# SamSamhuns/face_detection_and_recognition

Measured on AMD Instinct MI355X. Metric: faces/sec end-to-end (detect->embed->cosine-filter), 576x1024 batch=256, higher is better.
Workload: dtype f32 (bf16x6 split GEMMs)

## Files before the change

face_detection_and_recognition_amd/csrc/capi.cpp:

```cpp
#include <stdarg.h>
#include <stdio.h>
#include <stdlib.h>
#include <string.h>

#include "common.h"

static thread_local char g_hip_err[256] = "";

void fp_set_hip_error(hipError_t e) {
  const char* s = hipGetErrorString(e);
  strncpy(g_hip_err, s ? s : "unknown", sizeof(g_hip_err) - 1);
  g_hip_err[sizeof(g_hip_err) - 1] = 0;
}

static fp_knobs read_knobs() {
  fp_knobs k;
  k.resize_per_pixel = getenv("FP_RESIZE_PER_PIXEL") != nullptr;
  return k;
}
static fp_knobs g_knobs = read_knobs();
const fp_knobs& fp_get_knobs() { return g_knobs; }

bool fp_dry_run(const fp_launch& L, const char* fmt, ...) {
  if (!L.dry) return false;
  if (L.name) {
    va_list ap;
    va_start(ap, fmt);
    vsnprintf(L.name, FP_KERNEL_NAME_MAX, fmt, ap);
    va_end(ap);
  }
  return true;
}

static int launch_op(const fp_op& op, const fp_launch& L) {
  switch (op.kind) {
    case FP_OP_CONV: return fp_launch_conv(op, L);
    case FP_OP_DWCONV: return fp_launch_dwconv(op, L);
    case FP_OP_MAXPOOL: return fp_launch_maxpool(op, L);
    case FP_OP_UPSAMPLE2X: return fp_launch_upsample2x(op, L);
    case FP_OP_COPY: return fp_launch_copy(op, L);
    case FP_OP_L2NORM: return fp_launch_l2norm(op, L);
    case FP_OP_BLAZEBLOCK: return fp_launch_blazeblock(op, L);
    case FP_OP_DWPW: return (op.flags & FP_OPF_SPLIT3) ? fp_launch_dwpwx6(op, L) : fp_launch_dwpw(op, L);
    case FP_OP_DWBLOCK: return (op.flags & FP_OPF_SPLIT3) ? fp_launch_dwblock_x6(op, L) : fp_launch_dwblock(op, L);
    case FP_OP_BLAZEPAIR: return op.stride == 2 ? fp_launch_blazepair_s2(op, L) : fp_launch_blazepair(op, L);
    case FP_OP_BLAZECHAIN: return fp_launch_blazechain(op, L);
    case FP_OP_SHUFDOWN: return fp_launch_shufdown(op, L);
    case FP_OP_SHUFUNIT: return fp_launch_shufunit(op, L);
    case FP_OP_YSTEM2: return fp_launch_ystem2(op, L);
    case FP_OP_YSTEM: return fp_launch_ystem(op, L);
    case FP_OP_YSTEM_U8: return fp_launch_ystem_u8(op, L);
    case FP_OP_STEM_U8: return fp_launch_stem_u8(op, L);
    case FP_OP_EMBED_HEAD: return fp_launch_embed_head(op, L);
    case FP_OP_POOL_LRN: return fp_launch_pool_lrn(op, L);
    case FP_OP_CLS_HEAD: return fp_launch_cls_head(op, L);
    default: return FP_ERR_UNSUPPORTED;
  }
}

static int dry_run(const fp_op& op, char* name) {
  const fp_launch L = {nullptr, nullptr, nullptr, 0, nullptr, true, name};
  return launch_op(op, L);
}

extern "C" {

int fp_abi_version(void) { return FP_ABI_VERSION; }

void fp_debug_reload_env(void) { g_knobs = read_knobs(); }

const char* fp_last_hip_error(void) { return g_hip_err; }

static unsigned fastdiv_host(unsigned n, fp_divisor d) { return (unsigned)(((unsigned long long)n * d.mul) >> 32) >> d.shift; }

int fp_selftest(void) {
  auto check = [&](unsigned d) -> bool {
    const fp_divisor dv = fp_make_divisor(d);
    const unsigned nmax = 0x7fffffffu, qmax = nmax / d;
    const unsigned qs[] = {0u, 1u, 2u, qmax / 3, qmax / 2, qmax - 1, qmax};
    for (unsigned q : qs) {
      const unsigned long long lo = (unsigned long long)q * d;
      const unsigned long long cand[] = {lo, lo + 1, lo + d - 1, lo + d / 2};
      for (unsigned long long n64 : cand) {
        if (n64 > nmax) continue;
        const unsigned n = (unsigned)n64;
        if (fastdiv_host(n, dv) != n / d) {
          snprintf(g_hip_err, sizeof(g_hip_err), "fp_fastdiv(%u, %u) = %u, expected %u", n, d, fastdiv_host(n, dv), n / d);
          return false;
        }
      }
    }
    if (fastdiv_host(nmax, dv) != nmax / d) {
      snprintf(g_hip_err, sizeof(g_hip_err), "fp_fastdiv(%u, %u) wrong at the top of the range", nmax, d);
      return false;
    }
    return true;
  };
  for (unsigned d = 2; d <= 4096; ++d)
    if (!check(d)) return FP_ERR_INVALID_ARG;
  const unsigned big[] = {4097u, 12321u, 16384u, 65535u, 65536u, 65537u, 1000003u, 16777216u, 123456789u, 1u << 30, (1u << 30) + 1u};
  for (unsigned d : big)
    if (!check(d)) return FP_ERR_INVALID_ARG;
  return FP_OK;
}

const char* fp_strerror(int status) {
  switch (status) {
    case FP_OK: return "ok";
    case FP_ERR_INVALID_ARG: return "invalid argument";
    case FP_ERR_BOUNDS: return "op touches memory outside the arena or weight blob";
    case FP_ERR_UNSUPPORTED: return "unsupported op or parameter combination";
    case FP_ERR_LAUNCH: return "HIP kernel launch failed";
    case FP_ERR_ALIGNMENT: return "channel count / stride / offset not a multiple of 4 floats";
    default: return "unknown status";
  }
}

static bool span_ok(int64_t off, int64_t extent, size_t limit) {
  return off >= 0 && extent >= 0 && (uint64_t)(off + extent) <= (uint64_t)limit;
}

static int validate_op(const fp_op& op, size_t weight_floats, size_t arena_floats) {
  if (op.N <= 0 || op.H <= 0 || op.W <= 0 || op.Cin <= 0) return FP_ERR_INVALID_ARG;
  const bool spatial = op.kind != FP_OP_L2NORM && op.kind != FP_OP_COPY;
  const int OH = spatial ? op.OH : op.H, OW = spatial ? op.OW : op.W;
  if (OH <= 0 || OW <= 0) return FP_ERR_INVALID_ARG;
  const bool ext_in = op.kind == FP_OP_YSTEM_U8 || op.kind == FP_OP_STEM_U8;
  const int Cout = (op.kind == FP_OP_CONV || op.kind == FP_OP_BLAZEBLOCK || op.kind == FP_OP_DWPW ||
                    op.kind == FP_OP_DWBLOCK || op.kind == FP_OP_BLAZEPAIR || op.kind == FP_OP_BLAZECHAIN || op.kind == FP_OP_YSTEM ||
                    op.kind == FP_OP_SHUFDOWN || op.kind == FP_OP_SHUFUNIT || op.kind == FP_OP_YSTEM2 || op.kind == FP_OP_EMBED_HEAD ||
                    op.kind == FP_OP_CLS_HEAD || ext_in) ? op.Cout : op.Cin;
  if (op.kind != FP_OP_DWBLOCK && op.kind != FP_OP_BLAZECHAIN && op.kind != FP_OP_SHUFDOWN && op.kind != FP_OP_SHUFUNIT &&
      op.kind != FP_OP_POOL_LRN && op.Cmid != 0)
    return FP_ERR_INVALID_ARG;
  if (op.kind == FP_OP_POOL_LRN && op.Cout != op.Cin) return FP_ERR_INVALID_ARG;
  if (op.row_lo != 0 || op.row_end != 0) {
    if (op.kind != FP_OP_BLAZEPAIR && op.kind != FP_OP_STEM_U8) return FP_ERR_UNSUPPORTED;
    if (op.row_lo < 0 || op.row_end <= op.row_lo || op.row_end > OH) return FP_ERR_INVALID_ARG;
  }
  if (Cout <= 0 || op.out_cmul < 1 || op.in_ld < op.Cin) return FP_ERR_INVALID_ARG;
  if (op.flags & ~(FP_OPF_IN_ROWPAD | FP_OPF_OUT_ROWPAD | FP_OPF_IN_C3 | FP_OPF_SPLIT3 | FP_OPF_IN_DW | FP_OPF_IN_UP2 | FP_OPF_OUT_DW |
                   FP_OPF_OUT_L2))
    return FP_ERR_INVALID_ARG;
  if ((op.flags & FP_OPF_OUT_L2) && op.kind != FP_OP_EMBED_HEAD) return FP_ERR_INVALID_ARG;
  if (op.flags & FP_OPF_OUT_DW) {
    if (op.kind != FP_OP_CONV) return FP_ERR_INVALID_ARG;
    if (!span_ok(op.slope_off, 13 * (int64_t)op.Cout, weight_floats)) return FP_ERR_BOUNDS;
    if (!span_ok(op.w_off, fp_stemdw_w_floats(op), weight_floats)) return FP_ERR_BOUNDS;
  }
  if (op.flags & FP_OPF_IN_UP2) {
    if (op.kind != FP_OP_CONV || !(op.flags & FP_OPF_SPLIT3)) return FP_ERR_INVALID_ARG;
    const int64_t up_ext = (int64_t)(op.N - 1) * op.res_ns + ((int64_t)op.res_H * op.res_W - 1) * op.res_ld + op.res_C;
    if (!span_ok(op.res_off, up_ext, arena_floats)) return FP_ERR_BOUNDS;
  }
  if ((op.flags & FP_OPF_IN_DW) && (op.kind != FP_OP_DWBLOCK || !(op.flags & FP_OPF_SPLIT3))) return FP_ERR_INVALID_ARG;
  if ((op.flags & FP_OPF_SPLIT3) && op.kind != FP_OP_DWBLOCK && op.kind != FP_OP_CONV && op.kind != FP_OP_DWPW && op.kind != FP_OP_BLAZECHAIN &&
      op.kind != FP_OP_SHUFDOWN && op.kind != FP_OP_SHUFUNIT && op.kind != FP_OP_YSTEM2 && op.kind != FP_OP_STEM_U8)
    return FP_ERR_INVALID_ARG;
  if ((op.flags & FP_OPF_IN_C3) && (op.Cin != 4 || (op.kind != FP_OP_CONV && op.kind != FP_OP_YSTEM)))
    return FP_ERR_INVALID_ARG;
  const bool in_rp = (op.flags & FP_OPF_IN_ROWPAD) != 0, out_rp = (op.flags & FP_OPF_OUT_ROWPAD) != 0;
  if (in_rp && op.kind != FP_OP_BLAZEBLOCK && op.kind != FP_OP_BLAZEPAIR) return FP_ERR_UNSUPPORTED;
  if (out_rp && !(op.kind == FP_OP_BLAZEBLOCK || op.kind == FP_OP_BLAZEPAIR || op.kind == FP_OP_STEM_U8 || op.kind == FP_OP_COPY ||
                  op.kind == FP_OP_CONV))
    return FP_ERR_UNSUPPORTED;
  if (out_rp && (op.out_cmul != 1 || op.out_ld != Cout)) return FP_ERR_UNSUPPORTED;
  if (op.kind == FP_OP_CONV || op.kind == FP_OP_DWCONV || op.kind == FP_OP_MAXPOOL || op.kind == FP_OP_BLAZEBLOCK ||
      op.kind == FP_OP_DWPW || op.kind == FP_OP_DWBLOCK || op.kind == FP_OP_BLAZEPAIR || op.kind == FP_OP_BLAZECHAIN ||
      op.kind == FP_OP_YSTEM || op.kind == FP_OP_SHUFDOWN || op.kind == FP_OP_SHUFUNIT || op.kind == FP_OP_YSTEM2 ||
      op.kind == FP_OP_POOL_LRN || ext_in) {
    if (op.KH <= 0 || op.KW <= 0 || op.stride <= 0 || op.pad_t < 0 || op.pad_l < 0) return FP_ERR_INVALID_ARG;
    if ((int64_t)(OH - 1) * op.stride - op.pad_t >= op.H || (int64_t)(OW - 1) * op.stride - op.pad_l >= op.W)
      return FP_ERR_INVALID_ARG;
  }
  if (op.kind == FP_OP_YSTEM2) {
    const int64_t res_ext = (int64_t)(op.N - 1) * op.res_ns + ((int64_t)op.OH * op.OW - 1) * op.res_ld + op.res_C;
    if (!span_ok(op.res_off, res_ext, arena_floats)) return FP_ERR_BOUNDS;
  }
  const int rc = dry_run(op, nullptr);
  if (rc != FP_OK) return rc;
  if (in_rp) {
    const int64_t lead = (int64_t)(op.W + 2) * op.in_ld;
    if (op.in_ns < ((int64_t)(op.H + 2) * (op.W + 1) + 1) * op.in_ld) return FP_ERR_INVALID_ARG;
    if (op.in_off < lead || !span_ok(op.in_off - lead, (int64_t)op.N * op.in_ns, arena_floats)) return FP_ERR_BOUNDS;
  } else {
    const int64_t in_ext = (int64_t)(op.N - 1) * op.in_ns + ((int64_t)op.H * op.W - 1) * op.in_ld + op.Cin;
    if (!ext_in && !span_ok(op.in_off, in_ext, arena_floats)) return FP_ERR_BOUNDS;
  }
  if (ext_in && op.in_off < 0) return FP_ERR_INVALID_ARG;
  const int64_t out_ch = ((op.kind == FP_OP_CONV || op.kind == FP_OP_DWPW) && op.res_mode == FP_RES_SHUFFLE2)
                             ? 2 * (int64_t)Cout : Cout;
  if (out_rp) {
    const int64_t lead = (int64_t)(OW + 2) * op.out_ld;
    if (op.out_ns < ((int64_t)(OH + 2) * (OW + 1) + 1) * op.out_ld) return FP_ERR_INVALID_ARG;
    if (op.out_off < lead || !span_ok(op.out_off - lead, (int64_t)op.N * op.out_ns, arena_floats)) return FP_ERR_BOUNDS;
  } else {
    const int64_t out_ext =
        (int64_t)(op.N - 1) * op.out_ns + ((int64_t)OH * OW - 1) * op.out_ld + (out_ch - 1) * op.out_cmul + 1;
    if (!span_ok(op.out_off, out_ext, arena_floats)) return FP_ERR_BOUNDS;
  }
  if (op.in_ns < 0 || op.out_ns < 0) return FP_ERR_INVALID_ARG;

  if (op.kind == FP_OP_CONV || op.kind == FP_OP_BLAZEBLOCK || op.kind == FP_OP_STEM_U8) {
    int64_t wext;
    if (op.kind != FP_OP_BLAZEBLOCK) {
      const int64_t K = (int64_t)op.KH * op.KW * (op.kind == FP_OP_STEM_U8 ? 4 : op.Cin);
      wext = ((K + 7) / 8 * 8) * ((op.Cout + 31) / 32 * 32);
      if (op.flags & FP_OPF_SPLIT3)
        wext = op.kind == FP_OP_STEM_U8 ? 3 * 2 * 3 * 16 * 32 / 2 : fp_convx6_w_floats(op);
      if (op.flags & FP_OPF_OUT_DW) wext = fp_stemdw_w_floats(op);
    } else {
      wext = 9 * (int64_t)op.Cin;
      const int64_t pw = ((op.Cin + 7) / 8 * 8) * (int64_t)((op.Cout + 31) / 32 * 32);
      if (!span_ok(op.slope_off, pw, weight_floats)) return FP_ERR_BOUNDS;
      if (!span_ok(op.scale_off, op.Cin, weight_floats)) return FP_ERR_BOUNDS;
      if (!span_ok(op.bias_off, op.Cout, weight_floats)) return FP_ERR_BOUNDS;
    }
    if (!span_ok(op.w_off, wext, weight_floats)) return FP_ERR_BOUNDS;
  }
  if (op.kind == FP_OP_DWCONV) {
    if (!span_ok(op.w_off, (int64_t)op.KH * op.KW * op.Cin, weight_floats)) return FP_ERR_BOUNDS;
  }
  if (op.kind == FP_OP_DWPW) {
    if (!span_ok(op.w_off, 12 * (int64_t)op.Cin, weight_floats)) return FP_ERR_BOUNDS;
    const int64_t pw = (op.flags & FP_OPF_SPLIT3) ? fp_dwpwx6_w_floats(op) :
        ((op.Cin + 7) / 8 * 8) * (int64_t)((op.Cout + 31) / 32 * 32) + 2 * (int64_t)((op.Cout + 3) / 4 * 4);
    if (!span_ok(op.slope_off, pw, weight_floats)) return FP_ERR_BOUNDS;
    if (op.act != FP_ACT_NONE && op.act != FP_ACT_PRELU) return FP_ERR_INVALID_ARG;
    if (op.bias_off >= 0 && !span_ok(op.bias_off, (op.Cout + 3) / 4 * 4, weight_floats)) return FP_ERR_BOUNDS;
    if (op.act2 != FP_ACT_NONE && op.act2 != FP_ACT_SILU) return FP_ERR_INVALID_ARG;
  } else if (op.kind == FP_OP_SHUFDOWN) {
    if (!span_ok(op.w_off, fp_shufdown_w_floats(op), weight_floats)) return FP_ERR_BOUNDS;
  } else if (op.kind == FP_OP_YSTEM2) {
    if (!span_ok(op.w_off, fp_ystem2_w_floats(op), weight_floats)) return FP_ERR_BOUNDS;
  } else if (op.kind == FP_OP_SHUFUNIT) {
    if (!span_ok(op.w_off, fp_shufunit_w_floats(op), weight_floats)) return FP_ERR_BOUNDS;
  } else if (op.act2 != FP_ACT_NONE) {
    return FP_ERR_INVALID_ARG;
  }
  if (op.kind == FP_OP_BLAZEPAIR) {
    const int64_t pw2 = op.stride == 2 && op.Cout == 48 ? 2 * 768 : 768, c2 = op.stride == 2 ? op.Cout : 24;
    if (!span_ok(op.w_off, 2 * 9 * 24, weight_floats) || !span_ok(op.scale_off, 2 * 24, weight_floats) ||
        !span_ok(op.slope_off, 768 + pw2, weight_floats) || !span_ok(op.bias_off, 24 + c2, weight_floats))
      return FP_ERR_BOUNDS;
  }
  if (op.kind == FP_OP_BLAZECHAIN) {
    if (!span_ok(op.w_off, fp_blazechain_w_floats(op), weight_floats)) return FP_ERR_BOUNDS;
  }
  if (op.kind == FP_OP_DWBLOCK) {
    const bool x6 = (op.flags & FP_OPF_SPLIT3) != 0;
    if (!span_ok(op.w_off, x6 ? fp_dwblock_x6_we_floats(op) : (int64_t)op.Cin * op.Cmid, weight_floats)) return FP_ERR_BOUNDS;
    if (!span_ok(op.scale_off, 15 * (int64_t)op.Cmid, weight_floats)) return FP_ERR_BOUNDS;
    if ((op.flags & FP_OPF_IN_DW) && !span_ok(op.bias_off, 12 * (int64_t)op.Cin, weight_floats)) return FP_ERR_BOUNDS;
    if (!span_ok(op.slope_off, x6 ? fp_dwblock_x6_wp_floats(op) : (int64_t)op.Cmid * op.Cout + 2 * (int64_t)op.Cout, weight_floats))
      return FP_ERR_BOUNDS;
  }
  if (op.kind == FP_OP_YSTEM || op.kind == FP_OP_YSTEM_U8) {
    if (op.Cin != (ext_in ? 3 : 4) || op.res_C <= 0 || op.res_C > 32 || op.Cout > 32) return FP_ERR_UNSUPPORTED;
    if (op.res_H <= 0 || op.res_W <= 0 || op.res_ld < op.res_C || op.res_ns < 0) return FP_ERR_INVALID_ARG;
    const int nb2 = fp_ystem_nb2(op);
    if (!span_ok(op.w_off, 40 * 32, weight_floats) || !span_ok(op.bias_off, 32, weight_floats)) return FP_ERR_BOUNDS;
    if (op.scale_off >= 0 && !span_ok(op.scale_off, 32, weight_floats)) return FP_ERR_BOUNDS;
    if (!span_ok(op.slope_off, (int64_t)nb2 * 16 * (32 + 2), weight_floats)) return FP_ERR_BOUNDS;
    const int64_t res_ext = (int64_t)(op.N - 1) * op.res_ns + ((int64_t)(op.OH / 2) * (op.OW / 2) - 1) * op.res_ld + op.res_C;
    if (!span_ok(op.res_off, res_ext, arena_floats)) return FP_ERR_BOUNDS;
  }
  if (op.kind == FP_OP_CONV || op.kind == FP_OP_DWCONV || op.kind == FP_OP_STEM_U8) {
    if (op.scale_off >= 0 && !span_ok(op.scale_off, Cout, weight_floats)) return FP_ERR_BOUNDS;
    if (op.bias_off >= 0 && !span_ok(op.bias_off, Cout, weight_floats)) return FP_ERR_BOUNDS;
    if (op.slope_off >= 0 && !span_ok(op.slope_off, Cout, weight_floats)) return FP_ERR_BOUNDS;
    if (op.act == FP_ACT_PRELU && op.slope_off < 0) return FP_ERR_INVALID_ARG;
    if (op.act < FP_ACT_NONE || op.act > FP_ACT_SILU) return FP_ERR_INVALID_ARG;
  }
  if (op.kind == FP_OP_EMBED_HEAD) {
    if (!span_ok(op.w_off, (int64_t)op.Cout * op.Cin, weight_floats)) return FP_ERR_BOUNDS;
    if (op.scale_off >= 0 && !span_ok(op.scale_off, Cout, weight_floats)) return FP_ERR_BOUNDS;
    if (op.bias_off >= 0 && !span_ok(op.bias_off, Cout, weight_floats)) return FP_ERR_BOUNDS;
  }
  if (op.kind == FP_OP_POOL_LRN && op.Cmid) {
    if (!span_ok(op.w_off, 4, weight_floats)) return FP_ERR_BOUNDS;
  }
  if (op.kind == FP_OP_CLS_HEAD) {
    if (!span_ok(op.w_off, (int64_t)op.Cout * op.Cin, weight_floats)) return FP_ERR_BOUNDS;
    if (op.bias_off >= 0 && !span_ok(op.bias_off, Cout, weight_floats)) return FP_ERR_BOUNDS;
    if (op.res_off >= 0 && !span_ok(op.res_off, (int64_t)(op.N - 1) * op.res_ns + Cout, arena_floats)) return FP_ERR_BOUNDS;
  }
  if ((op.kind == FP_OP_CONV || op.kind == FP_OP_BLAZEBLOCK || op.kind == FP_OP_DWPW || op.kind == FP_OP_DWBLOCK) &&
      op.res_mode != FP_RES_NONE) {
    if (op.res_mode < FP_RES_NONE || op.res_mode > FP_RES_SHUFFLE2) return FP_ERR_INVALID_ARG;
    if (op.res_mode == FP_RES_SHUFFLE2 &&
        ((op.kind != FP_OP_CONV && op.kind != FP_OP_DWPW) || op.out_cmul != 1 || op.out_ld < 2 * op.Cout))
      return FP_ERR_INVALID_ARG;
    if (op.res_C <= 0 || op.res_ld < op.res_C || op.res_ns < 0) return FP_ERR_INVALID_ARG;
    int rh = OH, rw = OW;
    if (op.res_mode == FP_RES_POOL2_BEFORE_ACT) {
      rh = op.res_H;
      rw = op.res_W;
      if (rh < 2 * OH || rw < 2 * OW) return FP_ERR_INVALID_ARG;
    }
    const int64_t res_ext = (int64_t)(op.N - 1) * op.res_ns + ((int64_t)rh * rw - 1) * op.res_ld + op.res_C;
    if (!span_ok(op.res_off, res_ext, arena_floats)) return FP_ERR_BOUNDS;
  }
  return FP_OK;
}

const char* fp_op_kernel_name(const fp_op* op) {
  static thread_local char buf[FP_KERNEL_NAME_MAX];
  if (!op || dry_run(*op, buf) != FP_OK) return "?";
  return buf;
}

int fp_plan_validate(const fp_op* ops, int n_ops, size_t weight_floats, size_t arena_floats) {
  if (!ops || n_ops < 0) return FP_ERR_INVALID_ARG;
  for (int i = 0; i < n_ops; ++i) {
    int rc = validate_op(ops[i], weight_floats, arena_floats);
    if (rc != FP_OK) return rc;
  }
  return FP_OK;
}

// ... 100 lines not shown
```

face_detection_and_recognition_amd/csrc/common.h:

```cpp
#pragma once
#include <hip/hip_runtime.h>
#include <stdint.h>
#include "../../include/facepath.h"

typedef float f32x4 __attribute__((ext_vector_type(4)));
#define FP_MFMA_ORDER() __builtin_amdgcn_sched_barrier(0x7F6)

typedef float f32x16 __attribute__((ext_vector_type(16)));

#define FP_WAVE 64

__device__ __forceinline__ float fp_silu(float x) {
  const float e = __builtin_amdgcn_exp2f(-1.44269504088896341f * x);
  return x * __builtin_amdgcn_rcpf(1.0f + e);
}

struct fp_knobs {
  int resize_per_pixel;
};
const fp_knobs& fp_get_knobs();

void fp_set_hip_error(hipError_t e);

#define FP_CHECK_LAUNCH()                         \
  do {                                            \
    hipError_t e__ = hipGetLastError();           \
    if (e__ != hipSuccess) {                      \
      fp_set_hip_error(e__);                      \
      return FP_ERR_LAUNCH;                       \
    }                                             \
  } while (0)

struct fp_divisor {
  unsigned mul, shift;
};
static inline fp_divisor fp_make_divisor(unsigned d) {
  unsigned s = 0;
  while ((1ull << s) < d) ++s;
  fp_divisor r;
  r.mul = (unsigned)((1ull << (31 + s)) / d + 1ull);
  r.shift = s - 1;
  return r;
}
__device__ __forceinline__ unsigned fp_fastdiv(unsigned n, fp_divisor d) { return __umulhi(n, d.mul) >> d.shift; }

__device__ __forceinline__ unsigned fp_xcd_block() {
  const unsigned G = gridDim.x, b = blockIdx.x, q = G >> 3, rr = G & 7u, xcd = b & 7u, k = b >> 3;
  return (xcd < rr ? xcd * (q + 1) : rr * (q + 1) + (xcd - rr) * q) + k;
}

__device__ __forceinline__ long fp_uniform(long v) {
  const unsigned lo = __builtin_amdgcn_readfirstlane((unsigned)(unsigned long long)v);
  const unsigned hi = __builtin_amdgcn_readfirstlane((unsigned)((unsigned long long)v >> 32));
  return (long)(((unsigned long long)hi << 32) | lo);
}

static inline int fp_ceil_div(long a, long b) { return (int)((a + b - 1) / b); }

static inline int fp_window_bands(int rows, int N, int per_wg, int slots, int step_mul, int halo, int bmin, int min_rows) {
  int best = bmin;
  long best_cost = -1;
  for (int b = bmin; b == bmin || b <= rows / min_rows; ++b) {
    const long rounds = fp_ceil_div(fp_ceil_div((long)N * b, per_wg), slots);
    const long cost = rounds * ((long)step_mul * fp_ceil_div(rows, b) + halo);
    if (best_cost < 0 || cost < best_cost) best = b, best_cost = cost;
  }
  return best;
}
static inline long fp_round_up(long a, long b) { return (a + b - 1) / b * b; }

static inline bool fp_views_overlap(int N, long off_a, long ns_a, long hw_a, long ld_a, long c_a, long off_b, long ns_b,
                                    long hw_b, long ld_b, long c_b) {
  const long img_a = (hw_a - 1) * ld_a + c_a, img_b = (hw_b - 1) * ld_b + c_b;
  if (ns_a == ns_b) return off_a < off_b + img_b && off_b < off_a + img_a;
  return off_a < off_b + (long)(N - 1) * ns_b + img_b && off_b < off_a + (long)(N - 1) * ns_a + img_a;
}

#define FP_KERNEL_NAME_MAX 64
struct fp_launch {
  const float* weights;
  float* arena;
  const fp_ext* ext;
  int n_ext;
  hipStream_t s;
  bool dry;
  char* name;
};
bool fp_dry_run(const fp_launch& L, const char* fmt, ...) __attribute__((format(printf, 2, 3)));

int fp_launch_conv(const fp_op& op, const fp_launch& L);
int fp_launch_dwconv(const fp_op& op, const fp_launch& L);
int fp_launch_maxpool(const fp_op& op, const fp_launch& L);
int fp_launch_upsample2x(const fp_op& op, const fp_launch& L);
int fp_launch_copy(const fp_op& op, const fp_launch& L);
int fp_launch_l2norm(const fp_op& op, const fp_launch& L);
int fp_launch_embed_head(const fp_op& op, const fp_launch& L);
int fp_launch_pool_lrn(const fp_op& op, const fp_launch& L);
int fp_launch_cls_head(const fp_op& op, const fp_launch& L);
int fp_launch_blazeblock(const fp_op& op, const fp_launch& L);
int fp_launch_blazeblock_rowpad(const fp_op& op, const fp_launch& L);
int fp_launch_dwpw(const fp_op& op, const fp_launch& L);
int fp_launch_dwpwx6(const fp_op& op, const fp_launch& L);
int fp_launch_blazepair(const fp_op& op, const fp_launch& L);
int fp_launch_blazepair_s2(const fp_op& op, const fp_launch& L);
int fp_launch_blazechain(const fp_op& op, const fp_launch& L);
int fp_launch_dwblock(const fp_op& op, const fp_launch& L);
int fp_launch_dwblock_x6(const fp_op& op, const fp_launch& L);
int fp_launch_shufdown(const fp_op& op, const fp_launch& L);
int fp_launch_shufunit(const fp_op& op, const fp_launch& L);
int fp_launch_ystem2(const fp_op& op, const fp_launch& L);
int fp_launch_ystem(const fp_op& op, const fp_launch& L);
int fp_launch_ystem_u8(const fp_op& op, const fp_launch& L);
int fp_launch_stem_u8(const fp_op& op, const fp_launch& L);
int fp_launch_stemdw(const fp_op& op, const fp_launch& L);
bool fp_pwx6_eligible(const fp_op& op);
int fp_launch_pwx6(const fp_op& op, const fp_launch& L);
int fp_launch_convx6(const fp_op& op, const fp_launch& L);
bool fp_pws_eligible(const fp_op& op);
int fp_launch_pws(const fp_op& op, const fp_launch& L);
bool fp_stem_eligible(const fp_op& op);
int fp_launch_stem(const fp_op& op, const fp_launch& L);
bool fp_conv3_eligible(const fp_op& op);
int fp_launch_conv3(const fp_op& op, const fp_launch& L);

long fp_stemdw_w_floats(const fp_op& op);
long fp_convx6_w_floats(const fp_op& op);
long fp_dwpwx6_w_floats(const fp_op& op);
int64_t fp_blazechain_w_floats(const fp_op& op);
long fp_dwblock_x6_we_floats(const fp_op& op);
long fp_dwblock_x6_wp_floats(const fp_op& op);
long fp_shufdown_w_floats(const fp_op& op);
long fp_shufunit_w_floats(const fp_op& op);
long fp_ystem2_w_floats(const fp_op& op);
int fp_ystem_nb2(const fp_op& op);
```

face_detection_and_recognition_amd/csrc/stemdw.hip:

```cpp
#include "split.h"

namespace {

struct StemDwArgs {
  const float* in;
  float* out;
  const float* w;
  const float* scale;
  const float* bias;
  const float* slope;
  const float* dw;
  long in_ns, out_ns;
  int N;
};

constexpr int SD_H = 112, SD_OH = 56, SD_C = 64, SD_RB = 4, SD_NBAND = SD_OH / SD_RB;
constexpr int SD_IR = 2 * (SD_RB + 2) + 1;
constexpr int SD_IW = SD_H + 2;
constexpr int SD_CR = SD_RB + 2, SD_CW = SD_OH + 2;
constexpr int SD_LDC = 36;
constexpr int SD_IMG = SD_IR * SD_IW * 4, SD_C1 = SD_CR * SD_CW * SD_LDC, SD_PAR = 3 * SD_C, SD_DWP = 12 * SD_C;
constexpr int SD_LDS = 4 * (SD_IMG + SD_C1 + SD_PAR + SD_DWP);
constexpr int SD_PF = (SD_IR * SD_IW + 255) / 256;
static_assert(2 * SD_LDS <= 160 * 1024, "two workgroups per CU");

template <bool X6>
__global__ __launch_bounds__(256, 2) void stemdw_kernel(StemDwArgs p) {
  extern __shared__ __attribute__((aligned(16))) float smem[];
  float* Img = smem;
  float* C1 = Img + SD_IMG;
  float* Par = C1 + SD_C1;
  float* Dwp = Par + SD_PAR;
  const int tid = threadIdx.x, lane = tid & 63, wave = tid >> 6;
  const int lr = lane & 31, h = lane >> 5;
  const f32x4 z4 = {0.f, 0.f, 0.f, 0.f};
  const int ntiles = p.N * SD_NBAND, G = gridDim.x;

  if (tid < SD_PAR) Par[tid] = tid < SD_C ? p.scale[tid] : tid < 2 * SD_C ? p.bias[tid - SD_C] : p.slope[tid - 2 * SD_C];
  for (int i = tid; i < SD_DWP / 4; i += 256) *(f32x4*)&Dwp[i * 4] = *(const f32x4*)(p.dw + i * 4);
  if (tid < SD_CR * 2 * 8) {
    const int r = tid / 16, e = tid - r * 16, side = e >> 3, q = e & 7;
    *(f32x4*)&C1[((r * SD_CW) + (side ? SD_CW - 1 : 0)) * SD_LDC + q * 4] = z4;
  }
  f32x4 wf[X6 ? 1 : 2][X6 ? 1 : 5];
  fp_frag3 w3[X6 ? 4 : 1];
  const int l15 = lane & 15, q = lane >> 4;
  int koff[8];
  if (X6) {
    const unsigned short* wp = (const unsigned short*)p.w;
#pragma unroll
    for (int nt = 0; nt < 4; ++nt) {
      w3[nt].h = *(const u32x4*)(wp + ((nt * 3 + 0) * 16 + l15) * 32 + 8 * q);
      w3[nt].m = *(const u32x4*)(wp + ((nt * 3 + 1) * 16 + l15) * 32 + 8 * q);
      w3[nt].l = *(const u32x4*)(wp + ((nt * 3 + 2) * 16 + l15) * 32 + 8 * q);
    }
#pragma unroll
    for (int i = 0; i < 8; ++i) {
      const int k = 8 * q + i, tap = k < 27 ? k / 3 : 0, c = k < 27 ? k - tap * 3 : 0;
      koff[i] = ((tap / 3) * SD_IW + tap % 3) * 4 + c;
    }
  } else {
#pragma unroll
    for (int pass = 0; pass < 2; ++pass)
#pragma unroll
      for (int kq = 0; kq < 5; ++kq) {
        const int t = 2 * kq + h;
        const f32x4 v = *(const f32x4*)(p.w + ((long)(t < 9 ? t : 0) * SD_C + pass * 32 + lr) * 4);
        wf[pass][kq] = t < 9 ? v : z4;
      }
  }

  int srow[SD_PF], scol[SD_PF];
#pragma unroll
  for (int j = 0; j < SD_PF; ++j) {
    const int i = tid + 256 * j;
    srow[j] = i / SD_IW;
    scol[j] = i - srow[j] * SD_IW - 1;
  }
  f32x4 pre[SD_PF];
  unsigned premask = 0;
  auto issue_stage = [&](int tile) {
    const int img = tile / SD_NBAND, r0 = (tile - img * SD_NBAND) * SD_RB;
    const float* ib = p.in + (long)img * p.in_ns;
    premask = 0;
#pragma unroll
    for (int j = 0; j < SD_PF; ++j) {
      const int iy = 2 * r0 - 3 + srow[j], ix = scol[j];
      const bool ok = tid + 256 * j < SD_IR * SD_IW && (unsigned)iy < (unsigned)SD_H && (unsigned)ix < (unsigned)SD_H;
      pre[j] = *(const f32x4*)(ib + ((long)min(max(iy, 0), SD_H - 1) * SD_H + min(max(ix, 0), SD_H - 1)) * 4);
      if (ok) premask |= 1u << j;
    }
  };
  auto write_stage = [&]() {
#pragma unroll
    for (int j = 0; j < SD_PF; ++j)
      if (tid + 256 * j < SD_IR * SD_IW) *(f32x4*)&Img[(tid + 256 * j) * 4] = ((premask >> j) & 1u) ? pre[j] : z4;
  };

  const int c4 = tid & 7, col0 = tid >> 3;

  int tile = (int)fp_xcd_block();
  if (tile < ntiles) {
    issue_stage(tile);
    write_stage();
  }
  for (; tile < ntiles; tile += G) {
    const int img = tile / SD_NBAND, r0 = (tile - img * SD_NBAND) * SD_RB;
    float* ob = p.out + (long)img * p.out_ns;
    const bool more = tile + G < ntiles;
#pragma unroll
    for (int pass = 0; pass < 2; ++pass) {
      __syncthreads();
      if (pass == 0 && more) issue_stage(tile + G);
      if (X6) {
        constexpr int NT16 = SD_CR * SD_OH / 16, NOWN = (NT16 + 3) / 4;
#pragma unroll
        for (int t = 0; t < NOWN; ++t) {
          const int mt = wave + 4 * t;
          if (mt < NT16) {
            const int m = mt * 16 + l15;
            const int cy = m / SD_OH, cx = m - cy * SD_OH;
            const float* base = Img + ((cy * 2) * SD_IW + cx * 2) * 4;
            f32x4 lo, hi;
#pragma unroll
            for (int i = 0; i < 4; ++i) lo[i] = base[koff[i]], hi[i] = base[koff[4 + i]];
            const fp_frag3 pf = fp_split8(lo, hi);
            f32x4 acc0 = z4, acc1 = z4;
            fp_mfma_x6_2a(w3[2 * pass], w3[2 * pass + 1], pf.h, pf.m, pf.l, acc0, acc1);
            const bool inside = (unsigned)(r0 - 1 + cy) < (unsigned)SD_OH;
            float* dst = C1 + (cy * SD_CW + cx + 1) * SD_LDC + 4 * q;
#pragma unroll
            for (int nt = 0; nt < 2; ++nt) {
              const int ch = pass * 32 + 16 * nt + 4 * q;
              const f32x4 sc = *(const f32x4*)&Par[ch], bi = *(const f32x4*)&Par[SD_C + ch], sl = *(const f32x4*)&Par[2 * SD_C + ch];
              const f32x4 av = nt ? acc1 : acc0;
              f32x4 v;
#pragma unroll
              for (int e = 0; e < 4; ++e) {
                const float x = av[e] * sc[e] + bi[e];
                v[e] = x > 0.f ? x : __builtin_fmaf(x, sl[e], 0.0f);
              }
              *(f32x4*)(dst + 16 * nt) = inside ? v : z4;
            }
          }
        }
      } else {
  #pragma unroll 1
        for (int mt = wave; mt * 32 < SD_CR * SD_OH; mt += 4) {
          const int m = min(mt * 32 + lr, SD_CR * SD_OH - 1);
          const int cy = m / SD_OH, cx = m - cy * SD_OH;
          const float* base = Img + ((cy * 2) * SD_IW + cx * 2) * 4;
          f32x16 acc0, acc1;
  #pragma unroll
          for (int r = 0; r < 16; ++r) acc0[r] = 0.f, acc1[r] = 0.f;
  #pragma unroll
          for (int kq = 0; kq < 5; ++kq) {
            const int t = 2 * kq + h;
            const int tt = t < 9 ? t : 0;
            const int ky = tt / 3, kx = tt - ky * 3;
            const f32x4 a = *(const f32x4*)(base + (ky * SD_IW + kx) * 4);
  #pragma unroll
            for (int e = 0; e < 3; ++e) {
              if ((3 * kq + e) & 1) acc1 = __builtin_amdgcn_mfma_f32_32x32x2f32(wf[pass][kq][e], a[e], acc1, 0, 0, 0);
              else acc0 = __builtin_amdgcn_mfma_f32_32x32x2f32(wf[pass][kq][e], a[e], acc0, 0, 0, 0);
              FP_MFMA_ORDER();
            }
          }
          if (mt * 32 + lr < SD_CR * SD_OH) {
            const bool inside = (unsigned)(r0 - 1 + cy) < (unsigned)SD_OH;
            float* dst = C1 + (cy * SD_CW + cx + 1) * SD_LDC + 4 * h;
  #pragma unroll
            for (int j = 0; j < 4; ++j) {
              const int ch = pass * 32 + 8 * j + 4 * h;
              const f32x4 sc = *(const f32x4*)&Par[ch], bi = *(const f32x4*)&Par[SD_C + ch], sl = *(const f32x4*)&Par[2 * SD_C + ch];
              f32x4 v;
  #pragma unroll
              for (int e = 0; e < 4; ++e) {
                const float x = (acc0[4 * j + e] + acc1[4 * j + e]) * sc[e] + bi[e];
                v[e] = x > 0.f ? x : __builtin_fmaf(x, sl[e], 0.0f);
              }
              *(f32x4*)(dst + 8 * j) = inside ? v : z4;
            }
          }
        }
      }
      __syncthreads();
      if (pass == 1 && more) write_stage();

      {
        const float* dp = Dwp + pass * 32 + 4 * c4;
        f32x4 tap[9];
#pragma unroll
        for (int t = 0; t < 9; ++t) tap[t] = *(const f32x4*)(dp + t * SD_C);
        const f32x4 one = {1.f, 1.f, 1.f, 1.f};
        const f32x4 dsc = *(const f32x4*)(dp + 9 * SD_C), dbi = *(const f32x4*)(dp + 10 * SD_C);
        const f32x4 dsl = *(const f32x4*)(dp + 11 * SD_C) - one;
#pragma unroll
        for (int cp = 0; cp < 2; ++cp) {
          const int col = col0 + 32 * cp;
          if (col < SD_OH) {
            const float* base = C1 + col * SD_LDC + 4 * c4;
            f32x4 w0[3], w1[3], w2[3];
#pragma unroll
            for (int dx = 0; dx < 3; ++dx) {
              w0[dx] = *(const f32x4*)(base + dx * SD_LDC);
              w1[dx] = *(const f32x4*)(base + (SD_CW + dx) * SD_LDC);
            }
#pragma unroll
            for (int r = 0; r < SD_RB; ++r) {
#pragma unroll
              for (int dx = 0; dx < 3; ++dx) w2[dx] = *(const f32x4*)(base + ((r + 2) * SD_CW + dx) * SD_LDC);
              f32x4 a = w0[0] * tap[0];
              a += w0[1] * tap[1];
              a += w0[2] * tap[2];
#pragma unroll
              for (int dx = 0; dx < 3; ++dx) a += w1[dx] * tap[3 + dx];
#pragma unroll
              for (int dx = 0; dx < 3; ++dx) a += w2[dx] * tap[6 + dx];
              f32x4 v = a * dsc + dbi, ng;
#pragma unroll
              for (int i = 0; i < 4; ++i) ng[i] = __builtin_fminf(v[i], 0.f);
              v = ng * dsl + v;
              *(f32x4*)(ob + ((long)(r0 + r) * SD_OH + col) * SD_C + pass * 32 + 4 * c4) = v;
#pragma unroll
              for (int dx = 0; dx < 3; ++dx) {
                w0[dx] = w1[dx];
                w1[dx] = w2[dx];
              }
            }
          }
        }
      }
    }
  }
}

}

static bool stemdw_supported(const fp_op& op) {
  if (op.kind != FP_OP_CONV || !(op.flags & FP_OPF_OUT_DW) || !(op.flags & FP_OPF_IN_C3)) return false;
  if (op.flags & ~(FP_OPF_OUT_DW | FP_OPF_IN_C3 | FP_OPF_SPLIT3)) return false;
  if (op.H != SD_H || op.W != SD_H || op.OH != SD_OH || op.OW != SD_OH || op.Cin != 4 || op.Cout != SD_C) return false;
  if (op.KH != 3 || op.KW != 3 || op.stride != 2 || op.pad_t != 1 || op.pad_l != 1) return false;
  if (op.in_ld != 4 || op.out_ld != SD_C || op.out_cmul != 1) return false;
  if (op.act != FP_ACT_PRELU || op.res_mode != FP_RES_NONE) return false;
  if (op.scale_off < 0 || op.bias_off < 0 || op.slope_off < 0) return false;
  if (op.in_off % 4 || op.out_off % 4 || op.in_ns % 4 || op.out_ns % 4 || op.w_off % 4 || op.slope_off % 4) return false;
  return op.in_ns >= (long)SD_H * SD_H * 4 && op.out_ns >= (long)SD_OH * SD_OH * SD_C;
}

long fp_stemdw_w_floats(const fp_op& op) { return (op.flags & FP_OPF_SPLIT3) ? 4 * 3 * 16 * 32 / 2 : 40 * 64; }

int fp_launch_stemdw(const fp_op& op, const fp_launch& L) {
  if (!stemdw_supported(op)) return FP_ERR_UNSUPPORTED;
  const bool x6 = (op.flags & FP_OPF_SPLIT3) != 0;
  if (fp_dry_run(L, x6 ? "stemdw_kernel<true>" : "stemdw_kernel<false>")) return FP_OK;
  const float* weights = L.weights;
  float* arena = L.arena;
  const hipStream_t s = L.s;
  StemDwArgs a;
  a.in = arena + op.in_off;
  a.out = arena + op.out_off;
  a.w = weights + op.w_off;
  a.scale = weights + op.scale_off;
  a.bias = weights + op.bias_off;
  a.slope = weights + op.slope_off;
  a.dw = weights + op.slope_off + SD_C;
  a.in_ns = op.in_ns;
  a.out_ns = op.out_ns;
  a.N = op.N;
  const hipError_t ae = hipFuncSetAttribute(x6 ? (const void*)stemdw_kernel<true> : (const void*)stemdw_kernel<false>,
                                            hipFuncAttributeMaxDynamicSharedMemorySize, SD_LDS);
  if (ae != hipSuccess) {
    fp_set_hip_error(ae);
    return FP_ERR_LAUNCH;
  }
  const int ntiles = op.N * SD_NBAND, grid = ntiles < 512 ? ntiles : 512;
  if (x6) hipLaunchKernelGGL(stemdw_kernel<true>, dim3(grid), dim3(256), SD_LDS, s, a);
  else hipLaunchKernelGGL(stemdw_kernel<false>, dim3(grid), dim3(256), SD_LDS, s, a);
  FP_CHECK_LAUNCH();
  return FP_OK;
}
```

Measured before the change: 156,300.

## Stream stemdw bands in segments with ring-buffered conv rows and per-pass work items

Restructures the fused stem-conv plus depthwise kernel so each work item processes a contiguous segment of row bands for one channel half. Consecutive bands reuse the two halo rows of the first-stage output through a 6-row ring buffer, so only the 4 new rows (and 9 new input rows) are computed and loaded instead of recomputing the 6-row halo each band. Splitting the two channel passes into separate items doubles parallelism and halves the weight registers held per thread. A host heuristic chooses the segment length to balance halo savings against load balance across 512 slots, and env knobs can override segment length and grid size.

```diff
diff --git a/face_detection_and_recognition_amd/csrc/capi.cpp b/face_detection_and_recognition_amd/csrc/capi.cpp
--- a/face_detection_and_recognition_amd/csrc/capi.cpp
+++ b/face_detection_and_recognition_amd/csrc/capi.cpp
@@ -16,6 +16,10 @@
 static fp_knobs read_knobs() {
   fp_knobs k;
   k.resize_per_pixel = getenv("FP_RESIZE_PER_PIXEL") != nullptr;
+  const char* seg = getenv("FP_STEMDW_SEG");
+  const char* grid = getenv("FP_STEMDW_GRID");
+  k.stemdw_seg = seg ? atoi(seg) : 0;
+  k.stemdw_grid = grid ? atoi(grid) : 0;
   return k;
 }
 static fp_knobs g_knobs = read_knobs();
diff --git a/face_detection_and_recognition_amd/csrc/common.h b/face_detection_and_recognition_amd/csrc/common.h
--- a/face_detection_and_recognition_amd/csrc/common.h
+++ b/face_detection_and_recognition_amd/csrc/common.h
@@ -17,6 +17,8 @@
 
 struct fp_knobs {
   int resize_per_pixel;
+  int stemdw_seg;
+  int stemdw_grid;
 };
 const fp_knobs& fp_get_knobs();
 
diff --git a/face_detection_and_recognition_amd/csrc/stemdw.hip b/face_detection_and_recognition_amd/csrc/stemdw.hip
--- a/face_detection_and_recognition_amd/csrc/stemdw.hip
+++ b/face_detection_and_recognition_amd/csrc/stemdw.hip
@@ -12,29 +12,81 @@
   const float* dw;
   long in_ns, out_ns;
   int N;
+  int seg;
 };
 
 constexpr int SD_H = 112, SD_OH = 56, SD_C = 64, SD_RB = 4, SD_NBAND = SD_OH / SD_RB;
 constexpr int SD_IR = 2 * (SD_RB + 2) + 1;
+constexpr int SD_IRN = 2 * SD_RB + 1;
 constexpr int SD_IW = SD_H + 2;
 constexpr int SD_CR = SD_RB + 2, SD_CW = SD_OH + 2;
 constexpr int SD_LDC = 36;
 constexpr int SD_IMG = SD_IR * SD_IW * 4, SD_C1 = SD_CR * SD_CW * SD_LDC, SD_PAR = 3 * SD_C, SD_DWP = 12 * SD_C;
 constexpr int SD_LDS = 4 * (SD_IMG + SD_C1 + SD_PAR + SD_DWP);
 constexpr int SD_PF = (SD_IR * SD_IW + 255) / 256;
+constexpr int SD_SLOTS = 512;
 static_assert(2 * SD_LDS <= 160 * 1024, "two workgroups per CU");
+static_assert(SD_NBAND % 7 == 0 && SD_NBAND % 2 == 0, "segment lengths 1, 2, 7, 14");
+
+constexpr int sd_ring(int base, int yy) { return (base + yy) % SD_CR; }
+
+template <int BASE>
+__device__ __forceinline__ void sd_depthwise(const float* C1, const float* Dwp, float* ob, int r0, int pass, int c4, int col0) {
+  const float* dp = Dwp + pass * 32 + 4 * c4;
+  f32x4 tap[9];
+#pragma unroll
+  for (int t = 0; t < 9; ++t) tap[t] = *(const f32x4*)(dp + t * SD_C);
+  const f32x4 one = {1.f, 1.f, 1.f, 1.f};
+  const f32x4 dsc = *(const f32x4*)(dp + 9 * SD_C), dbi = *(const f32x4*)(dp + 10 * SD_C);
+  const f32x4 dsl = *(const f32x4*)(dp + 11 * SD_C) - one;
+#pragma unroll
+  for (int cp = 0; cp < 2; ++cp) {
+    const int col = col0 + 32 * cp;
+    if (col < SD_OH) {
+      const float* base = C1 + col * SD_LDC + 4 * c4;
+      f32x4 w0[3], w1[3], w2[3];
+#pragma unroll
+      for (int dx = 0; dx < 3; ++dx) {
+        w0[dx] = *(const f32x4*)(base + (sd_ring(BASE, 0) * SD_CW + dx) * SD_LDC);
+        w1[dx] = *(const f32x4*)(base + (sd_ring(BASE, 1) * SD_CW + dx) * SD_LDC);
+      }
+#pragma unroll
+      for (int r = 0; r < SD_RB; ++r) {
+#pragma unroll
+        for (int dx = 0; dx < 3; ++dx) w2[dx] = *(const f32x4*)(base + (sd_ring(BASE, r + 2) * SD_CW + dx) * SD_LDC);
+        f32x4 a = w0[0] * tap[0];
+        a += w0[1] * tap[1];
+        a += w0[2] * tap[2];
+#pragma unroll
+        for (int dx = 0; dx < 3; ++dx) a += w1[dx] * tap[3 + dx];
+#pragma unroll
+        for (int dx = 0; dx < 3; ++dx) a += w2[dx] * tap[6 + dx];
+        f32x4 v = a * dsc + dbi, ng;
+#pragma unroll
+        for (int i = 0; i < 4; ++i) ng[i] = __builtin_fminf(v[i], 0.f);
+        v = ng * dsl + v;
+        *(f32x4*)(ob + ((long)(r0 + r) * SD_OH + col) * SD_C + pass * 32 + 4 * c4) = v;
+#pragma unroll
+        for (int dx = 0; dx < 3; ++dx) {
+          w0[dx] = w1[dx];
+          w1[dx] = w2[dx];
+        }
+      }
+    }
+  }
+}
 
 template <bool X6>
 __global__ __launch_bounds__(256, 2) void stemdw_kernel(StemDwArgs p) {
   extern __shared__ __attribute__((aligned(16))) float smem[];
-  float* Img = smem;
-  float* C1 = Img + SD_IMG;
+  float* C1 = smem;
   float* Par = C1 + SD_C1;
   float* Dwp = Par + SD_PAR;
+  float* Img = Dwp + SD_DWP;
   const int tid = threadIdx.x, lane = tid & 63, wave = tid >> 6;
   const int lr = lane & 31, h = lane >> 5;
   const f32x4 z4 = {0.f, 0.f, 0.f, 0.f};
-  const int ntiles = p.N * SD_NBAND, G = gridDim.x;
+  const int S = p.seg, nseg = SD_NBAND / S, nitems = p.N * nseg * 2, G = gridDim.x;
 
   if (tid < SD_PAR) Par[tid] = tid < SD_C ? p.scale[tid] : tid < 2 * SD_C ? p.bias[tid - SD_C] : p.slope[tid - 2 * SD_C];
   for (int i = tid; i < SD_DWP / 4; i += 256) *(f32x4*)&Dwp[i * 4] = *(const f32x4*)(p.dw + i * 4);
@@ -42,196 +94,200 @@
     const int r = tid / 16, e = tid - r * 16, side = e >> 3, q = e & 7;
     *(f32x4*)&C1[((r * SD_CW) + (side ? SD_CW - 1 : 0)) * SD_LDC + q * 4] = z4;
   }
-  f32x4 wf[X6 ? 1 : 2][X6 ? 1 : 5];
-  fp_frag3 w3[X6 ? 4 : 1];
+  f32x4 wf[X6 ? 1 : 5];
+  fp_frag3 w3[X6 ? 2 : 1];
   const int l15 = lane & 15, q = lane >> 4;
   int koff[8];
   if (X6) {
-    const unsigned short* wp = (const unsigned short*)p.w;
-#pragma unroll
-    for (int nt = 0; nt < 4; ++nt) {
-      w3[nt].h = *(const u32x4*)(wp + ((nt * 3 + 0) * 16 + l15) * 32 + 8 * q);
-      w3[nt].m = *(const u32x4*)(wp + ((nt * 3 + 1) * 16 + l15) * 32 + 8 * q);
-      w3[nt].l = *(const u32x4*)(wp + ((nt * 3 + 2) * 16 + l15) * 32 + 8 * q);
-    }
 #pragma unroll
     for (int i = 0; i < 8; ++i) {
       const int k = 8 * q + i, tap = k < 27 ? k / 3 : 0, c = k < 27 ? k - tap * 3 : 0;
       koff[i] = ((tap / 3) * SD_IW + tap % 3) * 4 + c;
     }
-  } else {
-#pragma unroll
-    for (int pass = 0; pass < 2; ++pass)
+  }
+  auto load_weights = [&](int pass) {
+    if (X6) {
+      const unsigned short* wp = (const unsigned short*)p.w;
+#pragma unroll
+      for (int nt = 0; nt < 2; ++nt) {
+        const int ct = 2 * pass + nt;
+        w3[nt].h = *(const u32x4*)(wp + ((ct * 3 + 0) * 16 + l15) * 32 + 8 * q);
+        w3[nt].m = *(const u32x4*)(wp + ((ct * 3 + 1) * 16 + l15) * 32 + 8 * q);
+        w3[nt].l = *(const u32x4*)(wp + ((ct * 3 + 2) * 16 + l15) * 32 + 8 * q);
+      }
+    } else {
 #pragma unroll
       for (int kq = 0; kq < 5; ++kq) {
         const int t = 2 * kq + h;
         const f32x4 v = *(const f32x4*)(p.w + ((long)(t < 9 ? t : 0) * SD_C + pass * 32 + lr) * 4);
-        wf[pass][kq] = t < 9 ? v : z4;
-      }
-  }
-
-  int srow[SD_PF], scol[SD_PF];
-#pragma unroll
-  for (int j = 0; j < SD_PF; ++j) {
-    const int i = tid + 256 * j;
-    srow[j] = i / SD_IW;
-    scol[j] = i - srow[j] * SD_IW - 1;
-  }
+        wf[kq] = t < 9 ? v : z4;
+      }
+    }
+  };
+
   f32x4 pre[SD_PF];
   unsigned premask = 0;
-  auto issue_stage = [&](int tile) {
-    const int img = tile / SD_NBAND, r0 = (tile - img * SD_NBAND) * SD_RB;
+  int pre_n = 0;
+  auto issue_stage = [&](int img, int band, bool first) {
     const float* ib = p.in + (long)img * p.in_ns;
+    const int y0 = 2 * SD_RB * band + (first ? -3 : 1);
+    pre_n = (first ? SD_IR : SD_IRN) * SD_IW;
     premask = 0;
-#pragma unroll
-    for (int j = 0; j < SD_PF; ++j) {
-      const int iy = 2 * r0 - 3 + srow[j], ix = scol[j];
-      const bool ok = tid + 256 * j < SD_IR * SD_IW && (unsigned)iy < (unsigned)SD_H && (unsigned)ix < (unsigned)SD_H;
-      pre[j] = *(const f32x4*)(ib + ((long)min(max(iy, 0), SD_H - 1) * SD_H + min(max(ix, 0), SD_H - 1)) * 4);
-      if (ok) premask |= 1u << j;
-    }
+    int ts = tid;
+    asm volatile("" : "+v"(ts));
+#pragma unroll
+    for (int j = 0; j < SD_PF; ++j)
+      if (256 * j < pre_n) {
+        const int i = ts + 256 * j, sr = i / SD_IW;
+        const int iy = y0 + sr, ix = i - sr * SD_IW - 1;
+        const bool ok = tid + 256 * j < pre_n && (unsigned)iy < (unsigned)SD_H && (unsigned)ix < (unsigned)SD_H;
+        pre[j] = *(const f32x4*)(ib + ((long)min(max(iy, 0), SD_H - 1) * SD_H + min(max(ix, 0), SD_H - 1)) * 4);
+        if (ok) premask |= 1u << j;
+      }
   };
   auto write_stage = [&]() {
+    int ts = tid;
+    asm volatile("" : "+v"(ts));
 #pragma unroll
     for (int j = 0; j < SD_PF; ++j)
-      if (tid + 256 * j < SD_IR * SD_IW) *(f32x4*)&Img[(tid + 256 * j) * 4] = ((premask >> j) & 1u) ? pre[j] : z4;
+      if (ts + 256 * j < pre_n) *(f32x4*)(Img + ts * 4 + 1024 * j) = ((premask >> j) & 1u) ? pre[j] : z4;
   };
 
   const int c4 = tid & 7, col0 = tid >> 3;
 
-  int tile = (int)fp_xcd_block();
-  if (tile < ntiles) {
-    issue_stage(tile);
+  struct Step {
+    int item, j, img, band0, pass;
+  };
+  auto decode = [&](Step& st) {
+    if (st.item < nitems) {
+      const int t = st.item >> 1;
+      st.pass = st.item & 1;
+      st.img = t / nseg;
+      st.band0 = (t - st.img * nseg) * S;
+    }
+  };
+  auto next_step = [&](const Step& st) {
+    Step nx = st;
+    if (++nx.j == S) {
+      nx.item += G, nx.j = 0;
+      decode(nx);
+    }
+    return nx;
+  };
+  Step cur = {(int)fp_xcd_block(), 0, 0, 0, 0};
+  decode(cur);
+  if (cur.item < nitems) {
+    issue_stage(cur.img, cur.band0, true);
     write_stage();
   }
-  for (; tile < ntiles; tile += G) {
-    const int img = tile / SD_NBAND, r0 = (tile - img * SD_NBAND) * SD_RB;
-    float* ob = p.out + (long)img * p.out_ns;
-    const bool more = tile + G < ntiles;
-#pragma unroll
-    for (int pass = 0; pass < 2; ++pass) {
-      __syncthreads();
-      if (pass == 0 && more) issue_stage(tile + G);
-      if (X6) {
-        constexpr int NT16 = SD_CR * SD_OH / 16, NOWN = (NT16 + 3) / 4;
-#pragma unroll
-        for (int t = 0; t < NOWN; ++t) {
-          const int mt = wave + 4 * t;
-          if (mt < NT16) {
-            const int m = mt * 16 + l15;
-            const int cy = m / SD_OH, cx = m - cy * SD_OH;
-            const float* base = Img + ((cy * 2) * SD_IW + cx * 2) * 4;
-            f32x4 lo, hi;
-#pragma unroll
-            for (int i = 0; i < 4; ++i) lo[i] = base[koff[i]], hi[i] = base[koff[4 + i]];
-            const fp_frag3 pf = fp_split8(lo, hi);
-            f32x4 acc0 = z4, acc1 = z4;
-            fp_mfma_x6_2a(w3[2 * pass], w3[2 * pass + 1], pf.h, pf.m, pf.l, acc0, acc1);
-            const bool inside = (unsigned)(r0 - 1 + cy) < (unsigned)SD_OH;
-            float* dst = C1 + (cy * SD_CW + cx + 1) * SD_LDC + 4 * q;
-#pragma unroll
-            for (int nt = 0; nt < 2; ++nt) {
-              const int ch = pass * 32 + 16 * nt + 4 * q;
-              const f32x4 sc = *(const f32x4*)&Par[ch], bi = *(const f32x4*)&Par[SD_C + ch], sl = *(const f32x4*)&Par[2 * SD_C + ch];
-              const f32x4 av = nt ? acc1 : acc0;
-              f32x4 v;
-#pragma unroll
-              for (int e = 0; e < 4; ++e) {
-                const float x = av[e] * sc[e] + bi[e];
-                v[e] = x > 0.f ? x : __builtin_fmaf(x, sl[e], 0.0f);
-              }
-              *(f32x4*)(dst + 16 * nt) = inside ? v : z4;
-            }
+  Step nx1 = next_step(cur);
+  if (nx1.item < nitems) issue_stage(nx1.img, nx1.band0 + nx1.j, nx1.j == 0);
+  int wpass = -1;
+  while (cur.item < nitems) {
+    const int pass = cur.pass, band = cur.band0 + cur.j, r0 = band * SD_RB;
+    const bool first = cur.j == 0;
+    float* ob = p.out + (long)cur.img * p.out_ns;
+    if (pass != wpass) {
+      load_weights(pass);
+      wpass = pass;
+    }
+    __syncthreads();
+    const int g0 = r0 + (first ? -1 : 1), s0 = (r0 + (first ? 0 : 2)) % SD_CR;
+    if (X6) {
+      auto conv_tile = [&](int mt) {
+        const int m = mt * 16 + l15;
+        const int cy = m / SD_OH, cx = m - cy * SD_OH;
+        const float* base = Img + ((cy * 2) * SD_IW + cx * 2) * 4;
+        f32x4 lo, hi;
+#pragma unroll
+        for (int i = 0; i < 4; ++i) lo[i] = base[koff[i]], hi[i] = base[koff[4 + i]];
+        const fp_frag3 pf = fp_split8(lo, hi);
+        f32x4 acc0 = z4, acc1 = z4;
+        fp_mfma_x6_2a(w3[0], w3[1], pf.h, pf.m, pf.l, acc0, acc1);
+        const bool inside = (unsigned)(g0 + cy) < (unsigned)SD_OH;
+        int sl = s0 + cy;
+        sl -= sl >= SD_CR ? SD_CR : 0;
+        float* dst = C1 + (sl * SD_CW + cx + 1) * SD_LDC + 4 * q;
+#pragma unroll
+        for (int nt = 0; nt < 2; ++nt) {
+          const int ch = pass * 32 + 16 * nt + 4 * q;
+          const f32x4 sc = *(const f32x4*)&Par[ch], bi = *(const f32x4*)&Par[SD_C + ch], sl4 = *(const f32x4*)&Par[2 * SD_C + ch];
+          const f32x4 av = nt ? acc1 : acc0;
+          f32x4 v;
+#pragma unroll
+          for (int e = 0; e < 4; ++e) {
+            const float x = av[e] * sc[e] + bi[e];
+            v[e] = x > 0.f ? x : __builtin_fmaf(x, sl4[e], 0.0f);
+          }
+          *(f32x4*)(dst + 16 * nt) = inside ? v : z4;
+        }
+      };
+      static_assert(SD_RB * SD_OH / 16 > 11 && SD_CR * SD_OH / 16 == 21, "tiles 0 .. 11 in every band, 0 .. 20 in a first band");
+      conv_tile(wave);
+      conv_tile(wave + 4);
+      conv_tile(wave + 8);
+      if (first) {
+        conv_tile(wave + 12);
+        conv_tile(wave + 16);
+        if (wave == 0) conv_tile(20);
+      } else if (wave < 2) {
+        conv_tile(wave + 12);
+      }
+    } else {
+      const int npix = (first ? SD_CR : SD_RB) * SD_OH;
+#pragma unroll 1
+      for (int mt = wave; mt * 32 < npix; mt += 4) {
+        const int m = min(mt * 32 + lr, npix - 1);
+        const int cy = m / SD_OH, cx = m - cy * SD_OH;
+        const float* base = Img + ((cy * 2) * SD_IW + cx * 2) * 4;
+        f32x16 acc0, acc1;
+#pragma unroll
+        for (int r = 0; r < 16; ++r) acc0[r] = 0.f, acc1[r] = 0.f;
+#pragma unroll
+        for (int kq = 0; kq < 5; ++kq) {
+          const int t = 2 * kq + h;
+          const int tt = t < 9 ? t : 0;
+          const int ky = tt / 3, kx = tt - ky * 3;
+          const f32x4 a = *(const f32x4*)(base + (ky * SD_IW + kx) * 4);
+#pragma unroll
+          for (int e = 0; e < 3; ++e) {
+            if ((3 * kq + e) & 1) acc1 = __builtin_amdgcn_mfma_f32_32x32x2f32(wf[kq][e], a[e], acc1, 0, 0, 0);
+            else acc0 = __builtin_amdgcn_mfma_f32_32x32x2f32(wf[kq][e], a[e], acc0, 0, 0, 0);
+            FP_MFMA_ORDER();
           }
         }
-      } else {
-  #pragma unroll 1
-        for (int mt = wave; mt * 32 < SD_CR * SD_OH; mt += 4) {
-          const int m = min(mt * 32 + lr, SD_CR * SD_OH - 1);
-          const int cy = m / SD_OH, cx = m - cy * SD_OH;
-          const float* base = Img + ((cy * 2) * SD_IW + cx * 2) * 4;
-          f32x16 acc0, acc1;
-  #pragma unroll
-          for (int r = 0; r < 16; ++r) acc0[r] = 0.f, acc1[r] = 0.f;
-  #pragma unroll
-          for (int kq = 0; kq < 5; ++kq) {
-            const int t = 2 * kq + h;
-            const int tt = t < 9 ? t : 0;
-            const int ky = tt / 3, kx = tt - ky * 3;
-            const f32x4 a = *(const f32x4*)(base + (ky * SD_IW + kx) * 4);
-  #pragma unroll
-            for (int e = 0; e < 3; ++e) {
-              if ((3 * kq + e) & 1) acc1 = __builtin_amdgcn_mfma_f32_32x32x2f32(wf[pass][kq][e], a[e], acc1, 0, 0, 0);
-              else acc0 = __builtin_amdgcn_mfma_f32_32x32x2f32(wf[pass][kq][e], a[e], acc0, 0, 0, 0);
-              FP_MFMA_ORDER();
+        if (mt * 32 + lr < npix) {
+          const bool inside = (unsigned)(g0 + cy) < (unsigned)SD_OH;
+          int sl = s0 + cy;
+          sl -= sl >= SD_CR ? SD_CR : 0;
+          float* dst = C1 + (sl * SD_CW + cx + 1) * SD_LDC + 4 * h;
+#pragma unroll
+          for (int jj = 0; jj < 4; ++jj) {
+            const int ch = pass * 32 + 8 * jj + 4 * h;
+            const f32x4 sc = *(const f32x4*)&Par[ch], bi = *(const f32x4*)&Par[SD_C + ch], sl4 = *(const f32x4*)&Par[2 * SD_C + ch];
+            f32x4 v;
+#pragma unroll
+            for (int e = 0; e < 4; ++e) {
+              const float x = (acc0[4 * jj + e] + acc1[4 * jj + e]) * sc[e] + bi[e];
+              v[e] = x > 0.f ? x : __builtin_fmaf(x, sl4[e], 0.0f);
             }
-          }
-          if (mt * 32 + lr < SD_CR * SD_OH) {
-            const bool inside = (unsigned)(r0 - 1 + cy) < (unsigned)SD_OH;
-            float* dst = C1 + (cy * SD_CW + cx + 1) * SD_LDC + 4 * h;
-  #pragma unroll
-            for (int j = 0; j < 4; ++j) {
-              const int ch = pass * 32 + 8 * j + 4 * h;
-              const f32x4 sc = *(const f32x4*)&Par[ch], bi = *(const f32x4*)&Par[SD_C + ch], sl = *(const f32x4*)&Par[2 * SD_C + ch];
-              f32x4 v;
-  #pragma unroll
-              for (int e = 0; e < 4; ++e) {
-                const float x = (acc0[4 * j + e] + acc1[4 * j + e]) * sc[e] + bi[e];
-                v[e] = x > 0.f ? x : __builtin_fmaf(x, sl[e], 0.0f);
-              }
-              *(f32x4*)(dst + 8 * j) = inside ? v : z4;
-            }
+            *(f32x4*)(dst + 8 * jj) = inside ? v : z4;
           }
         }
       }
-      __syncthreads();
-      if (pass == 1 && more) write_stage();
-
-      {
-        const float* dp = Dwp + pass * 32 + 4 * c4;
-        f32x4 tap[9];
-#pragma unroll
-        for (int t = 0; t < 9; ++t) tap[t] = *(const f32x4*)(dp + t * SD_C);
-        const f32x4 one = {1.f, 1.f, 1.f, 1.f};
-        const f32x4 dsc = *(const f32x4*)(dp + 9 * SD_C), dbi = *(const f32x4*)(dp + 10 * SD_C);
-        const f32x4 dsl = *(const f32x4*)(dp + 11 * SD_C) - one;
-#pragma unroll
-        for (int cp = 0; cp < 2; ++cp) {
-          const int col = col0 + 32 * cp;
-          if (col < SD_OH) {
-            const float* base = C1 + col * SD_LDC + 4 * c4;
-            f32x4 w0[3], w1[3], w2[3];
-#pragma unroll
-            for (int dx = 0; dx < 3; ++dx) {
-              w0[dx] = *(const f32x4*)(base + dx * SD_LDC);
-              w1[dx] = *(const f32x4*)(base + (SD_CW + dx) * SD_LDC);
-            }
-#pragma unroll
-            for (int r = 0; r < SD_RB; ++r) {
-#pragma unroll
-              for (int dx = 0; dx < 3; ++dx) w2[dx] = *(const f32x4*)(base + ((r + 2) * SD_CW + dx) * SD_LDC);
-              f32x4 a = w0[0] * tap[0];
-              a += w0[1] * tap[1];
-              a += w0[2] * tap[2];
-#pragma unroll
-              for (int dx = 0; dx < 3; ++dx) a += w1[dx] * tap[3 + dx];
-#pragma unroll
-              for (int dx = 0; dx < 3; ++dx) a += w2[dx] * tap[6 + dx];
-              f32x4 v = a * dsc + dbi, ng;
-#pragma unroll
-              for (int i = 0; i < 4; ++i) ng[i] = __builtin_fminf(v[i], 0.f);
-              v = ng * dsl + v;
-              *(f32x4*)(ob + ((long)(r0 + r) * SD_OH + col) * SD_C + pass * 32 + 4 * c4) = v;
-#pragma unroll
-              for (int dx = 0; dx < 3; ++dx) {
-                w0[dx] = w1[dx];
-                w1[dx] = w2[dx];
-              }
-            }
-          }
-        }
-      }
-    }
+    }
+    __syncthreads();
+    const Step nx2 = next_step(nx1);
+    if (nx1.item < nitems) write_stage();
+    if (nx2.item < nitems) issue_stage(nx2.img, nx2.band0 + nx2.j, nx2.j == 0);
+
+    const int phase = band % 3;
+    if (phase == 0) sd_depthwise<0>(C1, Dwp, ob, r0, pass, c4, col0);
+    else if (phase == 1) sd_depthwise<4>(C1, Dwp, ob, r0, pass, c4, col0);
+    else sd_depthwise<2>(C1, Dwp, ob, r0, pass, c4, col0);
+
+    cur = nx1;
+    nx1 = nx2;
   }
 }
 
@@ -251,10 +307,26 @@
 
 long fp_stemdw_w_floats(const fp_op& op) { return (op.flags & FP_OPF_SPLIT3) ? 4 * 3 * 16 * 32 / 2 : 40 * 64; }
 
+static int stemdw_segment(int N) {
+  const int lens[4] = {14, 7, 2, 1};
+  int best = 1;
+  long best_cost = -1;
+  for (int S : lens) {
+    const long items = (long)N * (SD_NBAND / S) * 2;
+    if (S > 1 && items < 2 * SD_SLOTS) continue;
+    const long cost = fp_ceil_div(items, SD_SLOTS) * (SD_RB * S + 2);
+    if (best_cost < 0 || cost < best_cost) best = S, best_cost = cost;
+  }
+  return best;
+}
+
 int fp_launch_stemdw(const fp_op& op, const fp_launch& L) {
   if (!stemdw_supported(op)) return FP_ERR_UNSUPPORTED;
   const bool x6 = (op.flags & FP_OPF_SPLIT3) != 0;
   if (fp_dry_run(L, x6 ? "stemdw_kernel<true>" : "stemdw_kernel<false>")) return FP_OK;
+  const fp_knobs& knobs = fp_get_knobs();
+  const int S = knobs.stemdw_seg ? knobs.stemdw_seg : stemdw_segment(op.N);
+  if (S < 1 || SD_NBAND % S || knobs.stemdw_grid < 0) return FP_ERR_INVALID_ARG;
   const float* weights = L.weights;
   float* arena = L.arena;
   const hipStream_t s = L.s;
@@ -269,13 +341,16 @@
   a.in_ns = op.in_ns;
   a.out_ns = op.out_ns;
   a.N = op.N;
+  a.seg = S;
   const hipError_t ae = hipFuncSetAttribute(x6 ? (const void*)stemdw_kernel<true> : (const void*)stemdw_kernel<false>,
                                             hipFuncAttributeMaxDynamicSharedMemorySize, SD_LDS);
   if (ae != hipSuccess) {
     fp_set_hip_error(ae);
     return FP_ERR_LAUNCH;
   }
-  const int ntiles = op.N * SD_NBAND, grid = ntiles < 512 ? ntiles : 512;
+  const int nitems = op.N * (SD_NBAND / S) * 2;
+  int grid = nitems < SD_SLOTS ? nitems : SD_SLOTS;
+  if (knobs.stemdw_grid && knobs.stemdw_grid < grid) grid = knobs.stemdw_grid;
   if (x6) hipLaunchKernelGGL(stemdw_kernel<true>, dim3(grid), dim3(256), SD_LDS, s, a);
   else hipLaunchKernelGGL(stemdw_kernel<false>, dim3(grid), dim3(256), SD_LDS, s, a);
   FP_CHECK_LAUNCH();
```

Result: no change. 156,200 (-0.1%).
